# david8862/tf-keras-deeplabv3p-model-set

Measured on AMD Instinct MI355X. Metric: images/sec (513x513, 21-class) MobileNetV2-DeepLabV3+ OS=16 training step, higher is better.
Workload: dtype f32

## Files before the change

include/dl3p.h:

```cpp
#ifndef DL3P_H_
#define DL3P_H_

#include <stddef.h>
#include <stdint.h>

#ifdef __cplusplus
extern "C" {
#endif

#define DL3P_VERSION 100

enum {
  DL3P_OK = 0,
  DL3P_EINVAL = -1,
  DL3P_EUNSUPPORTED = -2,
  DL3P_ELAUNCH = -3,
  DL3P_EWORKSPACE = -4
};

enum { DL3P_ACT_NONE = 0, DL3P_ACT_RELU = 1, DL3P_ACT_RELU6 = 2, DL3P_ACT_HSWISH = 3, DL3P_ACT_HSIGMOID = 4 };

#define DL3P_MAX_STAT_ROWS 2048

int dl3p_version(void);
// ... 247 lines not shown
                                 int M, int K, int N, void* stream);
int dl3p_dwconv2d_bwd_weight_slabs(const float* x, int ldx, const float* in_scale, const float* in_shift, int in_act,
                                   const float* dy, int lddy, float* workspace, size_t workspace_bytes, int* rows_out,
                                   int N, int H, int W, int C, int k, int stride, int rate, int pad_t, int pad_l,
                                   int Ho, int Wo, void* stream);
int dl3p_stem_conv_bwd_weight_slabs(const float* x, int ldx, const float* dy, int lddy, float* workspace,
                                    size_t workspace_bytes, int* rows_out, int N, int H, int W, int Cout, int pad_t,
                                    int pad_l, int Ho, int Wo, void* stream);
int dl3p_stem_conv_bwd_weight_slabs_bn(const float* x, int ldx, const float* g, int ldg, const float* z, int ldz,
                                       const float* bn_scale, const float* bn_shift, int bn_act, const float* save_mean,
                                       const float* save_invstd, const float* coef, float* workspace, size_t workspace_bytes,
                                       int* rows_out, int N, int H, int W, int Cout, int pad_t, int pad_l, int Ho, int Wo,
                                       void* stream);
int dl3p_conv2d_gemm_bwd_weight_slabs(const float* x, int ldx, const float* in_scale, const float* in_shift, int in_act,
                                      const float* dy, int lddy, float* workspace, size_t workspace_bytes, int* rows_out,
                                      int N, int H, int W, int Cin, int Cout, int k, int stride, int rate,
                                      int pad_t, int pad_l, int Ho, int Wo, void* stream);
int dl3p_pwconv_bwd_weight_bn_supported(int M, int K, int N);
int dl3p_pwconv_bwd_weight_slabs_bn(const float* x, int ldx, const float* in_scale, const float* in_shift, int in_act,
                                    const float* g, int ldg, const float* z, int ldz, const float* bn_scale,
                                    const float* bn_shift, int bn_act, const float* save_mean, const float* save_invstd,
                                    const float* coef, float* dz, int lddz, float* workspace, size_t workspace_bytes,
                                    int* rows_out, int M, int K, int N, void* stream);
int dl3p_dw_upsampled_input(const float* up_x, int up_ld, int up_h, int up_w, int up_C, void* stream);
int dl3p_dw_upsampled_input_supported(int role, int N, int H, int W, int C, int up_C, int k, int stride, int rate, int pad_t, int pad_l,
                                      int Ho, int Wo);
int dl3p_dwconv2d_bwd_weight_bn_supported(int N, int H, int W, int C, int k, int stride, int rate, int pad_t, int pad_l,
                                          int Ho, int Wo);
int dl3p_dwconv2d_bwd_weight_slabs_bn(const float* x, int ldx, const float* in_scale, const float* in_shift, int in_act,
                                      const float* g, int ldg, const float* z, int ldz, const float* bn_scale,
                                      const float* bn_shift, int bn_act, const float* save_mean, const float* save_invstd,
                                      const float* coef, float* dz, int lddz, float* workspace, size_t workspace_bytes,
                                      int* rows_out, int N, int H, int W, int C, int k, int stride, int rate, int pad_t,
                                      int pad_l, int Ho, int Wo, void* stream);
int dl3p_pwconv_bwd_weight_slabs_bf16(const void* x, int ldx, const float* in_scale, const float* in_shift, int in_act,
                                      const void* dy, int lddy, int dy_is_f32, float* workspace, size_t workspace_bytes,
                                      int* rows_out, int M, int K, int N, void* stream);
int dl3p_dwconv2d_bwd_weight_slabs_bf16(const void* x, int ldx, const float* in_scale, const float* in_shift, int in_act,
                                        const void* dy, int lddy, float* workspace, size_t workspace_bytes, int* rows_out,
                                        int N, int H, int W, int C, int k, int stride, int rate, int pad_t, int pad_l,
                                        int Ho, int Wo, void* stream);

int dl3p_sgd_momentum(float* w, float* v, const float* g, size_t n, const float* lr_dev, float momentum,
                      float l2, float grad_scale, const float* l2_elem, const float* lr_scale_elem, void* stream);

int dl3p_adam_step(float* w, float* m, float* v, const float* g, size_t n, const float* lr_dev,
// ... 182 lines not shown
```

tf-keras-deeplabv3p-model-set_amd/_lib.py:

```python
import ctypes
import os
import re

HERE = os.path.dirname(os.path.abspath(__file__))
HEADER = os.path.join(HERE, '..', 'include', 'dl3p.h')
LIBPATH = os.path.join(HERE, 'libdl3p.so')

_CT = {
    'const float*': ctypes.c_void_p, 'float*': ctypes.c_void_p,
    'const double*': ctypes.c_void_p, 'double*': ctypes.c_void_p,
    'const int64_t*': ctypes.c_void_p, 'int64_t*': ctypes.c_void_p,
    'void*': ctypes.c_void_p, 'const void*': ctypes.c_void_p, 'void**': ctypes.POINTER(ctypes.c_void_p), 'int*': ctypes.POINTER(ctypes.c_int), 'unsigned long long*': ctypes.c_void_p, 'int32_t*': ctypes.c_void_p, 'uint32_t*': ctypes.c_void_p, 'const unsigned char*': ctypes.c_void_p, 'unsigned char*': ctypes.c_void_p, 'uint8_t*': ctypes.c_void_p, 'const uint8_t*': ctypes.c_void_p, 'const int*': ctypes.c_void_p, 'float*': ctypes.c_void_p,
    'int': ctypes.c_int, 'float': ctypes.c_float, 'double': ctypes.c_double,
    'size_t': ctypes.c_size_t, 'uint64_t': ctypes.c_uint64,
    'const char*': ctypes.c_char_p, 'void': None,
}


def parse_header(path=HEADER):
    src = open(path).read()
    src = re.sub(r'/\*.*?\*/', '', src, flags=re.S)
    src = re.sub(r'^\s*#.*$', '', src, flags=re.M)
    src = re.sub(r'\benum\s*\{[^}]*\}\s*;', '', src)
    src = src.replace('extern "C" {', '')
# ... 13 lines not shown
    return protos


class Dl3pError(RuntimeError):
    pass


class Lib:
    def __init__(self, path=LIBPATH):
        if not os.path.exists(path):
            raise ImportError(
                'libdl3p.so not found at %s -- build it with `python __graft_entry__.py` '
                '(there is no CPU fallback for the HIP path)' % path)
        import torch
        self.cdll = ctypes.CDLL(path)
        self.protos = parse_header()
        for name, (ret, args) in self.protos.items():
            fn = getattr(self.cdll, name)
            fn.restype = _CT[ret]
            fn.argtypes = [_CT[a] for a in args]
            setattr(self, name[len('dl3p_'):], self._wrap(name, fn, ret))

    def _wrap(self, name, fn, ret):
        if ret != 'int' or name in ('dl3p_version', 'dl3p_device_cus', 'dl3p_head_train_supported', 'dl3p_head_train_rows_supported', 'dl3p_stem_conv_supported', 'dl3p_conv2d_gemm_supported', 'dl3p_reduce_rows_variant', 'dl3p_reduce_rows_block_elements', 'dl3p_pwconv_bwd_weight_bn_supported', 'dl3p_dwconv2d_bwd_weight_bn_supported', 'dl3p_pwconv_sb_supported', 'dl3p_pwconv_sb_pays', 'dl3p_pwconv_bwd_data_sb_apply_supported', 'dl3p_conv2d_gemm_sb_supported', 'dl3p_conv2d_gemm_sb_pays', 'dl3p_irb_supported', 'dl3p_pwconv_fwd_splitk_plan', 'dl3p_irb_bwd_supported', 'dl3p_get_option', 'dl3p_irb_get_plan', 'dl3p_irb_cov_rows_max', 'dl3p_dw_upsampled_input_supported', 'dl3p_conv_narrow_supported', 'dl3p_ghost_fwd_supported', 'dl3p_deconv2x2_supported', 'dl3p_grad_clip_block_elements'):
            return fn
        err = self.cdll.dl3p_last_error_string
        err.restype = ctypes.c_char_p

        def call(*a):
            rc = fn(*a)
            if rc != 0:
                raise Dl3pError('%s failed (%d): %s' % (name, rc, err().decode()))
            return rc
        call.raw = fn
        call.__name__ = name
        return call


_lib = None


def lib():
    global _lib
    if _lib is None:
        _lib = Lib(os.environ['DL3P_LIB_OVERRIDE']) if os.environ.get('DL3P_LIB_OVERRIDE') else Lib()
    return _lib
```

tf-keras-deeplabv3p-model-set_amd/csrc/options.h:

```cpp
#pragma once
#include "common.h"

enum OptGet { GET_NONE, GET_SET, GET_LATCHED, GET_LATCHED_GE0, GET_RESOLVED };

#define DL3P_OPTION_TABLE(X)                                                                                                  \
                                                                    \
  X(PW_SMALL_MIN_ROWS, GET_NONE, "pw_small_min_rows", "DL3P_PW_SMALL_MIN_ROWS", 1 << 17, -1, v < 0 ? (1 << 17) : v)           \
                                \
  X(GEMM_NT, GET_NONE, "gemm_nt", nullptr, 0, 0, (v >= 1 && v <= 8) ? v : 0)                                                  \
              \
  X(GEMM_MI, GET_NONE, "gemm_mi", "DL3P_GEMM_MI", 0, 0, (v == 1 || v == 2) ? v : 0)                                           \
  X(GEMM_PER_CU, GET_NONE, "gemm_per_cu", "DL3P_GEMM_PER_CU", 0, 0, v > 0 ? v : 0)                                            \
                                                                \
  X(GEMM_TUNED, GET_NONE, "gemm_tuned", "DL3P_GEMM_TUNED", 1, -1, v ? 1 : 0)                                                  \
                   \
  X(SB_PIPE, GET_RESOLVED, "sb_pipe", "DL3P_SB_PIPE", 0, -1, v ? 1 : 0)                                                       \
                                                        \
  X(SPLIT_WGRAD, GET_LATCHED, "split_wgrad", "DL3P_SPLIT_WGRAD", env_int("DL3P_SPLIT_GEMM", 1), -1, v ? 1 : 0)                \
           \
  X(SPLIT_WGRAD_TILE, GET_NONE, "split_wgrad_tile", nullptr, -1, -1, (v >= 0 && v <= 4) ? v : -1)                             \
  X(SPLIT_WGRAD_PER_CU, GET_NONE, "split_wgrad_per_cu", nullptr, 0, 0, v > 0 ? v : 0)                                         \
                                                        \
  X(SPLITK, GET_SET, "splitk", "DL3P_SPLITK", -1, -1, v)                                                                      \
                     \
  X(SB_WM, GET_NONE, "sb_wm", nullptr, 0, 0, (v >= -1 && v <= 2) ? v : 0)                                                     \
  X(SB_NT, GET_NONE, "sb_nt", nullptr, 0, 0, (v == 8 || v == 12 || v == 16) ? v : 0)                                          \
                                       \
  X(SB_RS, GET_SET, "sb_rs", "DL3P_SB_RS", -1, -1, v < 0 ? -1 : (v ? 1 : 0))                                                  \
                                        \
  X(SB3, GET_LATCHED_GE0, "sb3", "DL3P_SB3", -1, -1, v < 0 ? -1 : (v ? 1 : 0))                                                \
                                     \
  X(BF16_KG, GET_NONE, "bf16_kg", "DL3P_BF16_KG", 0, -1, (v == 0 || v == 1 || v == 2 || v == 4) ? v : -1)                     \
                        \
  X(CONV_SB, GET_SET, "conv_sb", "DL3P_CONV_SB", 1, -1, (v >= 0 && v <= 2) ? v : -1)                                          \
                                      \
  X(DW_PER_CU, GET_NONE, "dw_per_cu", nullptr, 0, 0, v > 0 ? v : 0)                                                           \
  X(DW_WANT, GET_NONE, "dw_want", "DL3P_DW_WANT", DL3P_NUM_CUS * 3 / 2, 0, v > 0 ? v : 0)                                     \
  X(DW_MAXTH, GET_NONE, "dw_maxth", "DL3P_DW_MAXTH", 16, 0, v > 0 ? v : 0)                                                    \
  X(DW_TW, GET_NONE, "dw_tw", nullptr, 0, 0, (v == 2 || v == 4) ? v : 0)                                                      \
  X(DW_TUNED, GET_NONE, "dw_tuned", "DL3P_DW_TUNED", 1, -1, v ? 1 : 0)                                                        \
                                                                                                               \
  X(WGRAD_TILE, GET_NONE, "wgrad_tile", "DL3P_WGRAD_TILE", -1, -1, (v >= 0 && v <= 3) ? v : -1)                               \
  X(WGRAD_PER_CU, GET_NONE, "wgrad_per_cu", "DL3P_WGRAD_PER_CU", 4, 0, v > 0 ? v : 0)

enum Opt {
#define X(id, get, name, env, def, unset, norm) OPT_##id,
  DL3P_OPTION_TABLE(X)
#undef X
  OPT_COUNT
};

struct OptState { int set, env; bool env_read; };
extern OptState g_opt[OPT_COUNT];
int opt_env_read(Opt id);

static constexpr int k_opt_unset[OPT_COUNT] = {
#define X(id, get, name, env, def, unset, norm) unset,
// ... 8 lines not shown
```

tf-keras-deeplabv3p-model-set_amd/executor.py:

```python
import collections
import contextlib
import ctypes
import zlib
import numpy as np
import torch

from ._lib import lib
from .exec_options import GHOST_ON_BY_DEFAULT, ExecOptions
from .graph import ACT_NONE, ACT_RELU

MAX_ROWS = 2048
GHOST_DEFAULT = {(16, 8), (16, 24), (48, 12), (24, 36), (72, 12)}
GHOST_MIN_ROWS = 0

CONV_KINDS = ('conv_pw', 'conv_dense', 'conv_dw')
(R_IRB_EXPAND, R_IRB_DW, R_GHOST_PW, R_GHOST_DW, R_PW, R_DW, R_STEM, R_NARROW, R_GEMM, R_IM2COL) = (
    'irb_expand', 'irb_dw', 'ghost_pw', 'ghost_dw', 'pw', 'dw', 'stem', 'narrow', 'gemm', 'im2col')
NO_FRONT_SUMS = (None, 0, None, None, ACT_NONE, None, None, None, None)
Folded = collections.namedtuple('Folded', 'g ldg z ldz scale shift act mean invstd coef')
FoldedDg = collections.namedtuple('FoldedDg', Folded._fields + ('dz', 'lddz'))


def split_gemm_enabled():
    return ExecOptions.from_env().split_gemm
# ... 1231 lines not shown
    def _begin_backward(self, T):
        T.ws, T.wsb = self.workspace.data_ptr(), self.workspace.numel() * 4
        for op in self.g.ops:
            if getattr(op, 'b', None) is not None and self._bias_grad(op) is None:
                self.store.view(op.b, self.store.G).zero_()
        bucket_edges = self._bucket_edges() if self.dist is not None else {}
        T.defer = self.sync_bn
        T.fuse = self._bn_fusion_map()
        if self.bf16:
            T.fuse = {c: b for c, b in T.fuse.items() if c.kind == 'conv_pw' and self._rows(c) > 64 and self.opts.bf16_fuse_bn_bwd}
        T.stage_off = self._sync_total
        T.readers = self._bn_readers()
        T.bn_of = {id(o.z): o for o in self.g.ops if o.kind == 'bn'}
        T.fuse_add = self._bn_fusion_through_adds(T.readers) if not self.bf16 else {}
        T.batch = self.opts.batched_wgrad
        T.batch_wgrad = T.batch and not T.defer
        if T.batch_wgrad and not self.bf16:
            need = max([self._rows(op) * (op.cout if op.kind == 'conv_pw' else op.c) for op in self.g.ops
                        if op.kind in ('conv_pw', 'conv_dw') and op not in self._irb_expand] or [0])
            T.dz_scratch = torch.zeros(need + 64, **self.f32)
        if T.batch:
            slab_need = 0
            for op in self.g.ops:
                if op.kind in CONV_KINDS and op.layer.trainable and self._slab_bytes(op):
                    slab_need += (self._slab_bytes(op) + 255) // 256 * 256
            T.slab_ws = torch.zeros(slab_need // 4 + 64, **self.f32) if slab_need else None
        return bucket_edges

    def _wgrad(self, P, fn, *args):
        if self._bt.defer:
            self._bt.deferred.append((fn, args, P.ctx))
        else:
            P.k(fn, *args)

    def _slab_region(self, nbytes):
        T = self._bt
        region = T.slab_ws.data_ptr() + 4 * T.slab_off
        T.slab_off += ((nbytes + 255) // 256 * 256) // 4
        return region

    def _wgrad_slabs(self, P, fn, n, dst, nbytes, before, after, up=None):
        T, L = self._bt, self.L
        region = self._slab_region(nbytes)

        def issue(P2):
            rows = ctypes.c_int(0)
            if up is not None:
                P2.k(L.dw_upsampled_input, *up)
# ... 13 lines not shown
            for op2 in later:
                if (op2.kind == 'bn' and op2 not in T.bn_done and op2.z.requires_grad and op2.bn.layer.trainable
                        and T.readers.get(op2) and T.readers[op2] <= T.processed and op2 not in T.fuse.values()):
                    self._bn_backward_done(P, op2)

    def _bn_backward_done(self, P, bn_op, fused_rows=None):
        with P.at(_op_label(bn_op)):
            self._bn_backward(P, bn_op, fused_rows=fused_rows)
        self._bt.bn_done.add(bn_op)

    def _front_sums_done(self, P, front, front_add, rows):
        if front is not None:
            self._bn_backward_done(P, front, fused_rows=rows)
        elif front_add is not None:
            self._bt.presums[front_add] = rows

    def _conv_backward(self, P, op):
        T, out, xt = self._bt, op.out, op.x.tensor
        dz, lddz = self.tptr(out, True), out.ld
        need_gx = xt.requires_grad or xt.root.requires_grad
        sums_left = None
        if op.kind == 'conv_pw' and out.id in T.folded_dg:
            dz, lddz, sums_left = self._dgrad_folded(P, op)
        if op.layer.trainable and T.batch and self._slab_bytes(op):
            dz, lddz = self._wgrad_slab(P, op, dz, lddz, need_gx)
        elif op.layer.trainable:
            self._wgrad_plain(P, op, dz, lddz)
        if sums_left is not None:
            self._front_sums_done(P, *sums_left)
        elif need_gx:
            self._dgrad(P, op, dz, lddz)

    def _dgrad_folded(self, P, op):
        f = self._bt.folded_dg.pop(op.out.id)
        gp, ldg, acc = self._gbuf_acc(op.x)
        wsp, pitch = self.store.sb_ptr(op, False)
        front, front_add = self._front_bn(op)
        rows = ctypes.c_int(0)
        sums = self._front_sums(front or front_add, self.partials if front is not None else self.partials2, rows)
        P.k(self.L.pwconv_bwd_data_sb_apply, *f, wsp, pitch, gp, ldg, acc, *self._mkn(op), *sums)
        return f.dz, f.lddz, (front, front_add, rows.value)

    def _wgrad_slab(self, P, op, dz, lddz, need_gx):
        T, L = self._bt, self.L
        r = self._bwd_route(op)
        x = self.vargs(op.x)
        f = T.folded.pop(op.out.id, None)
        if f is not None and r != R_STEM:
            dz, lddz = (T.dz_scratch.data_ptr(), op.cout if r == R_PW else op.c) if need_gx else (None, 0)
        bn = f is not None
        before = (*x, *f, dz, lddz) if bn else (*x, dz, lddz)
        if r == R_PW:
            fn, n, after = (L.pwconv_bwd_weight_slabs_bn if bn else L.pwconv_bwd_weight_slabs), op.cin * op.cout, self._mkn(op)
        elif r == R_DW:
# ... 393 lines not shown
            if fused_rows is None:
                P.k(L.bn_bwd_reduce_bf16 if self.bf16 else L.bn_bwd_reduce, g, ldg, zp, ldz, sp, hp, bn.act, mean, invstd,
                    part, ctypes.byref(rows), M, bn.C)
            P.k(L.bn_bwd_finalize, part, rows.value, None, bn.C, float(M), st.ptr(lp['gamma']),
                invstd, sp, 0, st.ptr(lp['gamma'], G), st.ptr(lp['beta'], G), coef)
            if self.sync_bn:
                off = T.stage_off
                T.stage_off += 2 * bn.C
                P.k(L.bn_reduce_partials, part, rows.value, 2 * bn.C, self.sync_stage[off:].data_ptr())
                T.pending.append((op, off, P.ctx))
                T.sync_g[op] = (g, ldg)
                return
        if not frozen and op in self._irb_bn:
            return
        if not frozen and self._folds_apply_dgrad(op):
            T.folded_dg[z.id] = FoldedDg(g, ldg, zp, ldz, sp, hp, bn.act, mean, invstd, coef, dzo, lddzo)
            return
        if not frozen and self._folds_apply(op):
            T.folded[z.id] = Folded(g, ldg, zp, ldz, sp, hp, bn.act, mean, invstd, coef)
            T.dz_not_kept.add(z.root.id)
            return
        P.k(L.bn_bwd_apply_bf16 if self.bf16 else L.bn_bwd_apply, g, ldg, zp, ldz, sp, hp, bn.act, mean, invstd, coef, dzo,
            lddzo, 0, M, bn.C)

    def _folds_apply_dgrad(self, bn_op):
        conv = getattr(bn_op, 'producer', None)
        if (self.bf16 or self.sync_bn or self.dist is not None or conv is None or conv.kind != 'conv_pw' or conv.out is not bn_op.z
                or self.opts.fold_apply == 'off' or not self.opts.fold_apply_dgrad
                or conv in self._irb_expand):
            return False
        xt = conv.x.tensor
        if not (xt.requires_grad or xt.root.requires_grad):
            return False
        M = self._rows(conv)
        front, front_add = self._front_bn(conv)
        front = front or front_add
        vt = getattr(conv.x, 'view_grad', None)
        ldg = vt.ld if vt is not None else xt.ld
        if M * max(xt.ld, ldg, bn_op.z.ld, conv.cout, front.z.ld if front is not None else 0) * 4 >= 2 ** 32:
            return False
        if not self.L.pwconv_bwd_data_sb_apply_supported(M, conv.cin, conv.cout, bn_op.bn.act, 1 if front is not None else 0):
            return False
        return self._use_sb(conv, False, front is not None)

    def _folds_apply(self, bn_op):
        conv = getattr(bn_op, 'producer', None)
# ... 355 lines not shown
```

tf-keras-deeplabv3p-model-set_amd/ops.py:

```python
import ctypes
import torch

from ._lib import lib, Dl3pError

ACT_NONE, ACT_RELU, ACT_RELU6, ACT_HSWISH, ACT_HSIGMOID = 0, 1, 2, 3, 4
MAX_STAT_ROWS = 2048


def _stream():
    return torch.cuda.current_stream().cuda_stream


def _pl(t):
    if t is None:
        return None, 0
    if not t.is_cuda or t.dtype != torch.float32:
        raise Dl3pError('dl3p ops need float32 tensors on the HIP device (got %s on %s)' % (t.dtype, t.device))
    if t.stride(-1) != 1:
        raise Dl3pError('channel dim must be contiguous')
    ld = t.stride(-2) if t.dim() >= 2 else t.shape[-1]
    for d in range(t.dim() - 2):
        if t.shape[d + 1] > 0 and t.stride(d) != t.stride(d + 1) * t.shape[d + 1]:
            raise Dl3pError('rows are not evenly strided: %s %s' % (tuple(t.shape), t.stride()))
    return t.data_ptr(), ld
# ... 192 lines not shown
    dp, ldd = _pl(dy)
    lib().pwconv_bwd_weight(xp, ldx, _p(in_scale), _p(in_shift), in_act, dp, ldd, _p(gw), _p(gb), _p(ws),
                            ws.numel() * 4, M, K, Nn, _stream())
    return (gw, gb) if with_bias else gw


def pwconv_bwd_weight_bn(x, g, z, bn, act, in_scale=None, in_shift=None, in_act=ACT_NONE, want_dz=True):
    K, Nn = x.shape[-1], g.shape[-1]
    M = _rows(x)
    need = lib().pwconv_bwd_weight_workspace(M, K, Nn)
    ws = torch.empty(need // 4, dtype=torch.float32, device=x.device)
    gw = torch.empty((K, Nn), dtype=torch.float32, device=x.device)
    dz = torch.empty(g.shape, dtype=torch.float32, device=x.device) if want_dz else None
    xp, ldx = _pl(x)
    gp, ldg = _pl(g)
    zp, ldz = _pl(z)
    dp, ldd = _pl(dz)
    rows = ctypes.c_int(0)
    lib().pwconv_bwd_weight_slabs_bn(xp, ldx, _p(in_scale), _p(in_shift), in_act, gp, ldg, zp, ldz, _p(bn.scale), _p(bn.shift),
                                     act, _p(bn.mean), _p(bn.invstd), _p(bn.coef), dp, ldd or 0, _p(ws), ws.numel() * 4,
                                     ctypes.byref(rows), M, K, Nn, _stream())
    lib().reduce_rows(_p(ws), rows.value, K * Nn, _p(gw), 0, _stream())
    return gw, dz


def conv2d_fwd(x, w, stride=1, rate=1, padding='same', in_scale=None, in_shift=None, in_act=ACT_NONE, out=None,
               partials=None):
    N, H, W, Cin = x.shape
    k, _, _, Cout = w.shape
    Ho, Wo, pt, pl = conv_geometry(H, W, k, stride, rate, padding)
    y = out if out is not None else torch.empty((N, Ho, Wo, Cout), dtype=torch.float32, device=x.device)
    xp, ldx = _pl(x)
    yp, ldy = _pl(y)
    rows = ctypes.c_int(0)
    lib().conv2d_fwd(xp, ldx, _p(in_scale), _p(in_shift), in_act, _p(w), yp, ldy, _p(partials), ctypes.byref(rows),
                     N, H, W, Cin, Cout, k, stride, rate, pt, pl, Ho, Wo, _stream())
    return (y, rows.value) if partials is not None else y


def conv2d_bwd_weight(x, dy, k, stride=1, rate=1, padding='same', in_scale=None, in_shift=None, in_act=ACT_NONE):
    N, H, W, Cin = x.shape
    Cout = dy.shape[-1]
    Ho, Wo, pt, pl = conv_geometry(H, W, k, stride, rate, padding)
    need = lib().conv2d_bwd_weight_workspace(N, Ho, Wo, Cin, Cout, k)
    ws = torch.empty(need // 4, dtype=torch.float32, device=x.device)
    gw = torch.empty((k, k, Cin, Cout), dtype=torch.float32, device=x.device)
# ... 1050 lines not shown
```

Baseline: 1360.

## Fuse narrow pointwise conv backward: weight grad, data grad and BN stats in one kernel

Adds a fused HIP kernel for pointwise convolutions with small output channel counts. In one pass over the rows it applies the own BN backward, accumulates the weight gradient (and optional bias gradient) into per-block slabs, computes the input gradient with the weights held in LDS, and gathers the front BN statistics. The executor routes eligible conv_pw ops to it by default. This drops separate wgrad and dgrad launches and repeated reads of activations and gradients, at the cost of more LDS and register pressure and extra slab workspace.

```diff
diff --git a/include/dl3p.h b/include/dl3p.h
--- a/include/dl3p.h
+++ b/include/dl3p.h
@@ -293,6 +293,17 @@
                                     const float* bn_shift, int bn_act, const float* save_mean, const float* save_invstd,
                                     const float* coef, float* dz, int lddz, float* workspace, size_t workspace_bytes,
                                     int* rows_out, int M, int K, int N, void* stream);
+int dl3p_pwconv_bwd_narrow_supported(int M, int K, int N, int in_act, int own_act, int has_front, int has_bias, int accumulate,
+                                     int ld_max);
+int dl3p_pwconv_bwd_narrow_pays(int M, int K, int N);
+size_t dl3p_pwconv_bwd_narrow_workspace(int M, int K, int N, int ldw);
+int dl3p_pwconv_bwd_narrow(const float* z_in, int ldx, const float* in_scale, const float* in_shift, int in_act,
+                           const float* g, int ldg, const float* z_own, int ldz_own, const float* bn_scale,
+                           const float* bn_shift, int bn_act, const float* save_mean, const float* save_invstd,
+                           const float* coef, const float* w, int ldw, float* gx, int ldgx, int accumulate,
+                           const float* front_mean, const float* front_invstd, float* front_partials,
+                           int* front_rows_out, int with_bias, float* workspace, size_t workspace_bytes,
+                           int* rows_out, int M, int K, int N, void* stream);
 int dl3p_dw_upsampled_input(const float* up_x, int up_ld, int up_h, int up_w, int up_C, void* stream);
 int dl3p_dw_upsampled_input_supported(int role, int N, int H, int W, int C, int up_C, int k, int stride, int rate, int pad_t, int pad_l,
                                       int Ho, int Wo);
diff --git a/tf-keras-deeplabv3p-model-set_amd/_lib.py b/tf-keras-deeplabv3p-model-set_amd/_lib.py
--- a/tf-keras-deeplabv3p-model-set_amd/_lib.py
+++ b/tf-keras-deeplabv3p-model-set_amd/_lib.py
@@ -59,7 +59,7 @@
             setattr(self, name[len('dl3p_'):], self._wrap(name, fn, ret))
 
     def _wrap(self, name, fn, ret):
-        if ret != 'int' or name in ('dl3p_version', 'dl3p_device_cus', 'dl3p_head_train_supported', 'dl3p_head_train_rows_supported', 'dl3p_stem_conv_supported', 'dl3p_conv2d_gemm_supported', 'dl3p_reduce_rows_variant', 'dl3p_reduce_rows_block_elements', 'dl3p_pwconv_bwd_weight_bn_supported', 'dl3p_dwconv2d_bwd_weight_bn_supported', 'dl3p_pwconv_sb_supported', 'dl3p_pwconv_sb_pays', 'dl3p_pwconv_bwd_data_sb_apply_supported', 'dl3p_conv2d_gemm_sb_supported', 'dl3p_conv2d_gemm_sb_pays', 'dl3p_irb_supported', 'dl3p_pwconv_fwd_splitk_plan', 'dl3p_irb_bwd_supported', 'dl3p_get_option', 'dl3p_irb_get_plan', 'dl3p_irb_cov_rows_max', 'dl3p_dw_upsampled_input_supported', 'dl3p_conv_narrow_supported', 'dl3p_ghost_fwd_supported', 'dl3p_deconv2x2_supported', 'dl3p_grad_clip_block_elements'):
+        if ret != 'int' or name in ('dl3p_version', 'dl3p_device_cus', 'dl3p_head_train_supported', 'dl3p_head_train_rows_supported', 'dl3p_stem_conv_supported', 'dl3p_conv2d_gemm_supported', 'dl3p_reduce_rows_variant', 'dl3p_reduce_rows_block_elements', 'dl3p_pwconv_bwd_weight_bn_supported', 'dl3p_pwconv_bwd_narrow_supported', 'dl3p_pwconv_bwd_narrow_pays', 'dl3p_dwconv2d_bwd_weight_bn_supported', 'dl3p_pwconv_sb_supported', 'dl3p_pwconv_sb_pays', 'dl3p_pwconv_bwd_data_sb_apply_supported', 'dl3p_conv2d_gemm_sb_supported', 'dl3p_conv2d_gemm_sb_pays', 'dl3p_irb_supported', 'dl3p_pwconv_fwd_splitk_plan', 'dl3p_irb_bwd_supported', 'dl3p_get_option', 'dl3p_irb_get_plan', 'dl3p_irb_cov_rows_max', 'dl3p_dw_upsampled_input_supported', 'dl3p_conv_narrow_supported', 'dl3p_ghost_fwd_supported', 'dl3p_deconv2x2_supported', 'dl3p_grad_clip_block_elements'):
             return fn
         err = self.cdll.dl3p_last_error_string
         err.restype = ctypes.c_char_p
diff --git a/tf-keras-deeplabv3p-model-set_amd/csrc/options.h b/tf-keras-deeplabv3p-model-set_amd/csrc/options.h
--- a/tf-keras-deeplabv3p-model-set_amd/csrc/options.h
+++ b/tf-keras-deeplabv3p-model-set_amd/csrc/options.h
@@ -33,6 +33,8 @@
   X(BF16_KG, GET_NONE, "bf16_kg", "DL3P_BF16_KG", 0, -1, (v == 0 || v == 1 || v == 2 || v == 4) ? v : -1)                     \
                         \
   X(CONV_SB, GET_SET, "conv_sb", "DL3P_CONV_SB", 1, -1, (v >= 0 && v <= 2) ? v : -1)                                          \
+                                                                                                              \
+  X(PW_NARROW, GET_SET, "pw_narrow", "DL3P_PW_NARROW", 1, -1, (v >= 0 && v <= 2) ? v : -1)                                    \
                                       \
   X(DW_PER_CU, GET_NONE, "dw_per_cu", nullptr, 0, 0, v > 0 ? v : 0)                                                           \
   X(DW_WANT, GET_NONE, "dw_want", "DL3P_DW_WANT", DL3P_NUM_CUS * 3 / 2, 0, v > 0 ? v : 0)                                     \
diff --git a/tf-keras-deeplabv3p-model-set_amd/csrc/pw_narrow_bwd.hip b/tf-keras-deeplabv3p-model-set_amd/csrc/pw_narrow_bwd.hip
--- /dev/null
+++ b/tf-keras-deeplabv3p-model-set_amd/csrc/pw_narrow_bwd.hip
@@ -0,0 +1,439 @@
+#include <algorithm>
+#include <initializer_list>
+#include "common.h"
+#include "options.h"
+
+typedef float f32x4 __attribute__((ext_vector_type(4)));
+
+struct NarrowParams {
+  const float* X; int ldx; const float* scale; const float* shift; int act;
+  const float* G; int ldg;
+  const float* Z; int ldz;
+  const float* b_scale; const float* b_shift; const float* b_mean; const float* b_invstd; const float* b_coef; int b_act;
+  const float* W; int ldw;
+  float* GX; int ldgx;
+  const float* f_mean; const float* f_invstd; float* partials;
+  float* slabs; float* bias_slabs;
+  int M, K, N, S, R;
+};
+
+template <int KT, int NTN, int WAVES, bool BNA, bool BNB, bool BIAS>
+__global__ __launch_bounds__(64 * WAVES, (KT == 4 && (NTN == 2 || (BNA && BNB))) ? 2 : 3) void pw_narrow_bwd_kernel(NarrowParams p) {
+  constexpr int KS = 16 * KT, NP = 16 * NTN;
+  constexpr int XP = KS + 4, DP = NP + 4;
+  constexpr int WAVE_FLOATS = 16 * (XP + DP);
+  extern __shared__ __attribute__((aligned(16))) float nb_lds[];
+  const int WP = p.K + 4;
+  float* Wt = nb_lds;
+  float* sc_s = Wt + NP * WP;
+  float* sh_s = sc_s + p.K;
+  float* mu_s = sh_s + p.K;
+  float* is_s = mu_s + (BNB ? p.K : 0);
+  float* cf_s = is_s + (BNB ? p.K : 0);
+  float* wave0 = cf_s + (BNA ? 5 * NP : 0);
+  const int nthreads = blockDim.x;
+  const int t = threadIdx.x, l = t & 63, w = t >> 6, l15 = l & 15, q = l >> 4;
+  const int stream = w / p.S, slice = w - stream * p.S;
+  const int k0 = slice * KS;
+  float* Xs = wave0 + w * WAVE_FLOATS;
+  float* Ds = Xs + 16 * XP;
+  for (int idx = t; idx < NP * p.K; idx += nthreads) {
+    const int k = idx / NP, n = idx - k * NP;
+    Wt[n * WP + k] = n < p.N ? p.W[(size_t)k * p.ldw + n] : 0.f;
+  }
+  for (int i = t; i < p.K; i += nthreads) {
+    sc_s[i] = p.scale ? p.scale[i] : 1.f;
+    sh_s[i] = p.scale ? p.shift[i] : 0.f;
+    if (BNB) { mu_s[i] = p.f_mean[i]; is_s[i] = p.f_invstd[i]; }
+  }
+  if (BNA) {
+    for (int i = t; i < NP; i += nthreads) {
+      const bool in = i < p.N;
+      const float c0 = in ? p.b_coef[i] : 0.f, c1 = in ? p.b_coef[p.N + i] : 0.f, c2 = in ? p.b_coef[2 * p.N + i] : 0.f;
+      const float bc = in ? c0 * p.b_invstd[i] * c2 : 0.f;
+      cf_s[i] = c0;
+      cf_s[NP + i] = bc;
+      cf_s[2 * NP + i] = in ? bc * p.b_mean[i] - c0 * c1 : 0.f;
+      cf_s[3 * NP + i] = (in && p.b_scale) ? p.b_scale[i] : 1.f;
+      cf_s[4 * NP + i] = (in && p.b_shift) ? p.b_shift[i] : 0.f;
+    }
+  }
+  __syncthreads();
+
+  uint32_t xg[KT], gg[NTN], zg[BNA ? NTN : 1];
+  bool nok[NTN][4];
+#pragma unroll
+  for (int kt = 0; kt < KT; ++kt) xg[kt] = (uint32_t)(k0 + 16 * kt + 4 * q) * 4u;
+#pragma unroll
+  for (int nt = 0; nt < NTN; ++nt) {
+    const int n = 16 * nt + 4 * q;
+    gg[nt] = (uint32_t)(n < p.N ? n : 0) * 4u;
+    if (BNA) zg[nt] = gg[nt];
+#pragma unroll
+    for (int e = 0; e < 4; ++e) nok[nt][e] = n + e < p.N;
+  }
+  const float act_lo = p.act == DL3P_ACT_NONE ? -DL3P_INF : 0.f;
+  const float act_hi = (p.act == DL3P_ACT_NONE || p.act == DL3P_ACT_RELU) ? DL3P_INF : 6.f;
+
+  f32x4 acc[KT][NTN];
+#pragma unroll
+  for (int a = 0; a < KT; ++a)
+#pragma unroll
+    for (int b = 0; b < NTN; ++b) acc[a][b] = (f32x4){0.f, 0.f, 0.f, 0.f};
+  float4 st_s[BNB ? KT : 1], st_q[BNB ? KT : 1], bsum[BIAS ? NTN : 1];
+  if (BNB) {
+#pragma unroll
+    for (int i = 0; i < KT; ++i) { st_s[i] = zero4(); st_q[i] = zero4(); }
+  }
+  if (BIAS) {
+#pragma unroll
+    for (int i = 0; i < NTN; ++i) bsum[i] = zero4();
+  }
+
+  const int ntiles = (p.M + 15) >> 4;
+  const int nstreams = gridDim.x * p.R;
+  const int gs = blockIdx.x * p.R + stream;
+  const char* Xb = reinterpret_cast<const char*>(p.X);
+  const char* Gb = reinterpret_cast<const char*>(p.G);
+  const char* Zb = reinterpret_cast<const char*>(p.Z);
+  char* Ob = reinterpret_cast<char*>(p.GX);
+  float4 rx[KT], rg[NTN], rz[BNA ? NTN : 1];
+#define NB_PREFETCH_X(tile_)                                                                                   \
+  {                                                                                                            \
+    const uint32_t xb0 = (uint32_t)min(((tile_) << 4) + l15, p.M - 1) * (uint32_t)p.ldx * 4u;                  \
+    _Pragma("unroll") for (int i = 0; i < KT; ++i) rx[i] = *reinterpret_cast<const float4*>(Xb + (xb0 + xg[i]));   \
+  }
+#define NB_PREFETCH_G(tile_)                                                                                   \
+  {                                                                                                            \
+    const uint32_t prow = (uint32_t)min(((tile_) << 4) + l15, p.M - 1);                                        \
+    const uint32_t gb0 = prow * (uint32_t)p.ldg * 4u;                                                          \
+    _Pragma("unroll") for (int i = 0; i < NTN; ++i) rg[i] = *reinterpret_cast<const float4*>(Gb + (gb0 + gg[i]));  \
+    if (BNA) {                                                                                                 \
+      const uint32_t zb0 = prow * (uint32_t)p.ldz * 4u;                                                        \
+      _Pragma("unroll") for (int i = 0; i < NTN; ++i) rz[i] = *reinterpret_cast<const float4*>(Zb + (zb0 + zg[i])); \
+    }                                                                                                          \
+  }
+  NB_PREFETCH_X(min(gs, ntiles - 1))
+  NB_PREFETCH_G(min(gs, ntiles - 1))
+  for (int tile = gs; tile < ntiles; tile += nstreams) {
+    const int m0 = tile << 4;
+    const bool row_ok = m0 + l15 < p.M;
+    int cq = 4 * q;
+    asm volatile("" : "+v"(cq));
+    float4 xh[BNB ? KT : 1];
+    uint32_t dmask = 0;
+#pragma unroll
+    for (int kt = 0; kt < KT; ++kt) {
+      const float4 s4 = *reinterpret_cast<const float4*>(&sc_s[k0 + 16 * kt + cq]);
+      const float4 h4 = *reinterpret_cast<const float4*>(&sh_s[k0 + 16 * kt + cq]);
+      const float4 u = fma4(rx[kt], s4, h4);
+      const float4 v = make_float4(__builtin_amdgcn_fmed3f(u.x, act_lo, act_hi), __builtin_amdgcn_fmed3f(u.y, act_lo, act_hi),
+                                   __builtin_amdgcn_fmed3f(u.z, act_lo, act_hi), __builtin_amdgcn_fmed3f(u.w, act_lo, act_hi));
+      *reinterpret_cast<float4*>(&Xs[l15 * XP + 16 * kt + 4 * q]) = row_ok ? v : zero4();
+      if (BNB) {
+        const float4 mu = *reinterpret_cast<const float4*>(&mu_s[k0 + 16 * kt + cq]);
+        const float4 is = *reinterpret_cast<const float4*>(&is_s[k0 + 16 * kt + cq]);
+        const float4 zv = rx[kt];
+        xh[kt] = make_float4((zv.x - mu.x) * is.x, (zv.y - mu.y) * is.y, (zv.z - mu.z) * is.z, (zv.w - mu.w) * is.w);
+        dmask |= ((u.x > act_lo && u.x < act_hi) ? 1u : 0u) << (4 * kt);
+        dmask |= ((u.y > act_lo && u.y < act_hi) ? 1u : 0u) << (4 * kt + 1);
+        dmask |= ((u.z > act_lo && u.z < act_hi) ? 1u : 0u) << (4 * kt + 2);
+        dmask |= ((u.w > act_lo && u.w < act_hi) ? 1u : 0u) << (4 * kt + 3);
+        asm volatile("" : "+v"(xh[kt].x), "+v"(xh[kt].y), "+v"(xh[kt].z), "+v"(xh[kt].w));
+      }
+    }
+    if (BNB) asm volatile("" : "+v"(dmask));
+    float dz[NTN][4];
+#pragma unroll
+    for (int nt = 0; nt < NTN; ++nt) {
+      float4 v = rg[nt];
+      if (BNA) {
+        const int cf = 16 * nt + cq;
+        const float4 a4 = *reinterpret_cast<const float4*>(&cf_s[cf]);
+        const float4 c4 = *reinterpret_cast<const float4*>(&cf_s[NP + cf]);
+        const float4 d4 = *reinterpret_cast<const float4*>(&cf_s[2 * NP + cf]);
+        const float4 s4 = *reinterpret_cast<const float4*>(&cf_s[3 * NP + cf]);
+        const float4 h4 = *reinterpret_cast<const float4*>(&cf_s[4 * NP + cf]);
+        const float4 z = rz[nt];
+        const float4 u = fma4(z, s4, h4);
+        const int act = p.b_act;
+        v = make_float4(fmaf(a4.x, v.x * act_grad(u.x, act), fmaf(-c4.x, z.x, d4.x)),
+                        fmaf(a4.y, v.y * act_grad(u.y, act), fmaf(-c4.y, z.y, d4.y)),
+                        fmaf(a4.z, v.z * act_grad(u.z, act), fmaf(-c4.z, z.z, d4.z)),
+                        fmaf(a4.w, v.w * act_grad(u.w, act), fmaf(-c4.w, z.w, d4.w)));
+      }
+      dz[nt][0] = (row_ok && nok[nt][0]) ? v.x : 0.f;
+      dz[nt][1] = (row_ok && nok[nt][1]) ? v.y : 0.f;
+      dz[nt][2] = (row_ok && nok[nt][2]) ? v.z : 0.f;
+      dz[nt][3] = (row_ok && nok[nt][3]) ? v.w : 0.f;
+      const float4 d4v = make_float4(dz[nt][0], dz[nt][1], dz[nt][2], dz[nt][3]);
+      *reinterpret_cast<float4*>(&Ds[l15 * DP + 16 * nt + 4 * q]) = d4v;
+      if (BIAS) bsum[nt] = add4(bsum[nt], d4v);
+    }
+    NB_PREFETCH_X(min(tile + nstreams, ntiles - 1))
+    __builtin_amdgcn_sched_barrier(0);
+    {
+      float b[NTN][4];
+#pragma unroll
+      for (int nt = 0; nt < NTN; ++nt)
+#pragma unroll
+        for (int j = 0; j < 4; ++j) b[nt][j] = Ds[(4 * q + j) * DP + nt * 16 + l15];
+#pragma unroll
+      for (int kt = 0; kt < KT; ++kt) {
+        float a[4];
+#pragma unroll
+        for (int j = 0; j < 4; ++j) a[j] = Xs[(4 * q + j) * XP + kt * 16 + l15];
+#pragma unroll
+        for (int nt = 0; nt < NTN; ++nt)
+#pragma unroll
+          for (int j = 0; j < 4; ++j)
+            acc[kt][nt] = __builtin_amdgcn_mfma_f32_16x16x4f32(b[nt][j], a[j], acc[kt][nt], 0, 0, 0);
+      }
+    }
+    f32x4 gacc[KT];
+#pragma unroll
+    for (int kt = 0; kt < KT; ++kt) {
+      gacc[kt] = (f32x4){0.f, 0.f, 0.f, 0.f};
+#pragma unroll
+      for (int nt = 0; nt < NTN; ++nt)
+#pragma unroll
+        for (int j = 0; j < 4; ++j)
+          gacc[kt] = __builtin_amdgcn_mfma_f32_16x16x4f32(Wt[(nt * 16 + 4 * q + j) * WP + k0 + kt * 16 + l15], dz[nt][j], gacc[kt], 0, 0, 0);
+    }
+    __builtin_amdgcn_sched_barrier(0);
+    NB_PREFETCH_G(min(tile + nstreams, ntiles - 1))
+#pragma unroll
+    for (int kt = 0; kt < KT; ++kt) {
+      const float4 o = make_float4(gacc[kt][0], gacc[kt][1], gacc[kt][2], gacc[kt][3]);
+      if (BNB) {
+        const float4 d = make_float4((dmask >> (4 * kt)) & 1u ? o.x : 0.f, (dmask >> (4 * kt + 1)) & 1u ? o.y : 0.f,
+                                     (dmask >> (4 * kt + 2)) & 1u ? o.z : 0.f, (dmask >> (4 * kt + 3)) & 1u ? o.w : 0.f);
+        st_s[kt] = add4(st_s[kt], d);
+        st_q[kt] = fma4(d, xh[kt], st_q[kt]);
+      }
+      *reinterpret_cast<float4*>(&Xs[l15 * XP + 16 * kt + 4 * q]) = o;
+    }
+    const uint32_t ob0 = ((uint32_t)m0 * (uint32_t)p.ldgx + (uint32_t)k0) * 4u;
+    const int rows_here = p.M - m0;
+#pragma unroll
+    for (int i = 0; i < KT; ++i) {
+      const int f = l + 64 * i;
+      const int r = f / (KS / 4), c = f - r * (KS / 4);
+      if (r < rows_here)
+        st4(reinterpret_cast<float*>(Ob + (ob0 + ((uint32_t)r * (uint32_t)p.ldgx + (uint32_t)c * 4u) * 4u)),
+            *reinterpret_cast<const float4*>(&Xs[r * XP + c * 4]));
+    }
+  }
+#undef NB_PREFETCH_X
+#undef NB_PREFETCH_G
+
+  __syncthreads();
+  int t_end = threadIdx.x;
+  asm volatile("" : "+v"(t_end));
+  const int te = t_end, le = te & 63, we = te >> 6, l15e = le & 15, qe = le >> 4;
+  const int streame = we / p.S, slicee = we - streame * p.S;
+  const int k0e = slicee * KS;
+  float4* red = reinterpret_cast<float4*>(nb_lds);
+  if (streame > 0) {
+#pragma unroll
+    for (int kt = 0; kt < KT; ++kt)
+#pragma unroll
+      for (int nt = 0; nt < NTN; ++nt)
+        red[(((streame - 1) * p.S + slicee) * KT * NTN + kt * NTN + nt) * 64 + le] =
+            make_float4(acc[kt][nt][0], acc[kt][nt][1], acc[kt][nt][2], acc[kt][nt][3]);
+  }
+  __syncthreads();
+  if (streame == 0) {
+    float* slab = p.slabs + (size_t)blockIdx.x * p.K * p.ldw;
+#pragma unroll
+    for (int kt = 0; kt < KT; ++kt)
+#pragma unroll
+      for (int nt = 0; nt < NTN; ++nt) {
+        float4 v = make_float4(acc[kt][nt][0], acc[kt][nt][1], acc[kt][nt][2], acc[kt][nt][3]);
+        for (int r = 1; r < p.R; ++r) v = add4(v, red[(((r - 1) * p.S + slicee) * KT * NTN + kt * NTN + nt) * 64 + le]);
+        const int k = k0e + kt * 16 + l15e, n = nt * 16 + qe * 4;
+        if (n < p.ldw) st4(slab + (size_t)k * p.ldw + n, v);
+      }
+  }
+  if (BNB) {
+    float4* S4 = reinterpret_cast<float4*>(nb_lds);
+    const int k4 = p.K >> 2;
+#pragma unroll
+    for (int which = 0; which < 2; ++which) {
+      __syncthreads();
+#pragma unroll
+      for (int kt = 0; kt < KT; ++kt) S4[(streame * 16 + l15e) * k4 + ((k0e + 16 * kt) >> 2) + qe] = which ? st_q[kt] : st_s[kt];
+      __syncthreads();
+      if (te < k4) {
+        float4 sum = zero4();
+        for (int ww = 0; ww < p.R; ++ww)
+          for (int r = 0; r < 16; ++r) sum = add4(sum, S4[(ww * 16 + r) * k4 + te]);
+        st4(p.partials + ((size_t)blockIdx.x * 2 + which) * p.K + 4 * te, sum);
+      }
+    }
+  }
+  if (BIAS) {
+    __syncthreads();
+    float* bred = nb_lds;
+#pragma unroll
+    for (int nt = 0; nt < NTN; ++nt) {
+      float bv[4] = {bsum[nt].x, bsum[nt].y, bsum[nt].z, bsum[nt].w};
+#pragma unroll
+      for (int e = 0; e < 4; ++e) {
+        float s1 = bv[e];
+#pragma unroll
+        for (int d = 1; d < 16; d <<= 1) s1 += __shfl_xor(s1, d);
+        if (l15e == 0 && slicee == 0) bred[streame * NP + 16 * nt + 4 * qe + e] = s1;
+      }
+    }
+    __syncthreads();
+    for (int i = te; i < p.ldw; i += nthreads) {
+      float sum = bred[i];
+      for (int r = 1; r < p.R; ++r) sum += bred[r * NP + i];
+      p.bias_slabs[(size_t)blockIdx.x * p.ldw + i] = sum;
+    }
+  }
+}
+
+struct NarrowPlan { int kt, ntn, S, R, grid; size_t lds; };
+
+static int narrow_kt(int K) {
+  if (K == 32) return 2;
+  if (K % 48 == 0 && K <= 192) return 3;
+  if (K % 64 == 0 && K <= 256) return 4;
+  return 0;
+}
+
+static bool narrow_plan(int M, int K, int N, bool bna, bool bnb, NarrowPlan* pl) {
+  const int kt = narrow_kt(K);
+  if (M <= 0 || N < 1 || N > 32 || !kt) return false;
+  pl->kt = kt;
+  pl->ntn = N <= 16 ? 1 : 2;
+  pl->S = K / (16 * kt);
+  pl->R = pl->S <= 3 ? 4 : 1;
+  static const int per_cu_env = env_int("DL3P_PW_NARROW_PER_CU", 0);
+  const int per_cu = per_cu_env > 0 ? per_cu_env : (pl->R == 1 && kt == 3 ? 3 : 2);
+  int g = ceil_div(M, 16) / (pl->R * 2);
+  g = std::min(g, DL3P_NUM_CUS * per_cu);
+  g = std::min(g, DL3P_MAX_STAT_ROWS);
+  pl->grid = std::max(g, 1);
+  const int np = 16 * pl->ntn, ks = 16 * kt, waves = pl->S * pl->R;
+  const size_t stage = (size_t)np * (K + 4) + 2 * K + (bnb ? 2 * K : 0) + (bna ? 5 * np : 0) + (size_t)waves * 16 * (ks + 4 + np + 4);
+  const size_t red = std::max({(size_t)4 * (pl->R - 1) * pl->S * kt * pl->ntn * 64, (size_t)pl->R * 16 * K, (size_t)pl->R * np});
+  pl->lds = sizeof(float) * std::max(stage, red);
+  return true;
+}
+
+template <int KT, int NTN, int WAVES, bool BNA, bool BNB, bool BIAS>
+static void launch_narrow(const NarrowParams& p, const NarrowPlan& pl, hipStream_t st) {
+  static size_t attr_lds = 0;
+  if (pl.lds > attr_lds) {
+    (void)hipFuncSetAttribute(reinterpret_cast<const void*>(pw_narrow_bwd_kernel<KT, NTN, WAVES, BNA, BNB, BIAS>),
+                              hipFuncAttributeMaxDynamicSharedMemorySize, (int)pl.lds);
+    attr_lds = pl.lds;
+  }
+  dl3p_launch(pw_narrow_bwd_kernel<KT, NTN, WAVES, BNA, BNB, BIAS>, dim3(pl.grid), dim3(64 * WAVES), pl.lds, st, p);
+}
+
+template <int KT, int NTN, int WAVES>
+static void launch_narrow_modes(const NarrowParams& p, const NarrowPlan& pl, bool bna, bool bnb, bool bias, hipStream_t st) {
+  if (bias) {
+    if (bnb) launch_narrow<KT, NTN, WAVES, false, true, true>(p, pl, st);
+    else launch_narrow<KT, NTN, WAVES, false, false, true>(p, pl, st);
+  } else if (bna) {
+    if (bnb) launch_narrow<KT, NTN, WAVES, true, true, false>(p, pl, st);
+    else launch_narrow<KT, NTN, WAVES, true, false, false>(p, pl, st);
+  } else {
+    if (bnb) launch_narrow<KT, NTN, WAVES, false, true, false>(p, pl, st);
+    else launch_narrow<KT, NTN, WAVES, false, false, false>(p, pl, st);
+  }
+}
+
+template <int NTN>
+static bool launch_narrow_shape(const NarrowParams& p, const NarrowPlan& pl, bool bna, bool bnb, bool bias, hipStream_t st) {
+  switch (pl.kt * 100 + pl.S * pl.R) {
+    case 204: launch_narrow_modes<2, NTN, 4>(p, pl, bna, bnb, bias, st); return true;
+    case 304: launch_narrow_modes<3, NTN, 4>(p, pl, bna, bnb, bias, st); return true;
+    case 308: launch_narrow_modes<3, NTN, 8>(p, pl, bna, bnb, bias, st); return true;
+    case 312: launch_narrow_modes<3, NTN, 12>(p, pl, bna, bnb, bias, st); return true;
+    case 404: launch_narrow_modes<4, NTN, 4>(p, pl, bna, bnb, bias, st); return true;
+    case 408: launch_narrow_modes<4, NTN, 8>(p, pl, bna, bnb, bias, st); return true;
+    default: return false;
+  }
+}
+
+static bool narrow_act_ok(int act) { return act == DL3P_ACT_NONE || act == DL3P_ACT_RELU || act == DL3P_ACT_RELU6; }
+
+extern "C" int dl3p_pwconv_bwd_narrow_supported(int M, int K, int N, int in_act, int own_act, int has_front, int has_bias,
+                                                int accumulate, int ld_max) {
+  NarrowPlan pl;
+  if (!narrow_plan(M, K, N, own_act >= 0, has_front != 0, &pl)) return 0;
+  if (accumulate || !narrow_act_ok(in_act) || own_act > DL3P_ACT_HSIGMOID) return 0;
+  if (own_act >= 0 && has_bias) return 0;
+  if (ld_max < 0 || (unsigned long long)M * (unsigned long long)std::max(ld_max, std::max(K, 32)) * 4ull >= (1ull << 32)) return 0;
+  return 1;
+}
+
+extern "C" int dl3p_pwconv_bwd_narrow_pays(int M, int K, int N) {
+  const int mode = opt(OPT_PW_NARROW);
+  if (mode == 0) return 0;
+  if (mode == 2) return 1;
+  NarrowPlan pl;
+  return M >= (1 << 17) && narrow_plan(M, K, N, false, false, &pl) && pl.R == 4;
+}
+
+extern "C" size_t dl3p_pwconv_bwd_narrow_workspace(int M, int K, int N, int ldw) {
+  NarrowPlan pl;
+  if (!narrow_plan(M, K, N, false, false, &pl) || ldw < N || ldw > 16 * pl.ntn) return 0;
+  return (size_t)pl.grid * ((size_t)K * ldw + ldw) * sizeof(float);
+}
+
+extern "C" int dl3p_pwconv_bwd_narrow(const float* z_in, int ldx, const float* in_scale, const float* in_shift, int in_act,
+                                      const float* g, int ldg, const float* z_own, int ldz_own, const float* bn_scale,
+                                      const float* bn_shift, int bn_act, const float* save_mean, const float* save_invstd,
+                                      const float* coef, const float* w, int ldw, float* gx, int ldgx, int accumulate,
+                                      const float* front_mean, const float* front_invstd, float* front_partials,
+                                      int* front_rows_out, int with_bias, float* workspace, size_t workspace_bytes,
+                                      int* rows_out, int M, int K, int N, void* stream) {
+  const char* fn = "dl3p_pwconv_bwd_narrow";
+  const bool bna = z_own != nullptr, bnb = front_partials != nullptr;
+  const int n4 = (N + 3) / 4 * 4;
+  DL3P_CHECK_ARG(z_in && g && w && gx && workspace && rows_out && aligned16(z_in) && aligned16(g) && aligned16(w) && aligned16(gx) &&
+                 aligned16(workspace), "%s: null or misaligned operand", fn);
+  DL3P_CHECK_ARG(M > 0 && K > 0 && N > 0 && ldx >= K && ldgx >= K && ldg >= n4 && ldw >= N && ldw <= (N <= 16 ? 16 : 32) && ldx % 4 == 0 && ldgx % 4 == 0 &&
+                 ldg % 4 == 0 && ldw % 4 == 0, "%s: bad layout (M=%d K=%d N=%d ldx=%d ldgx=%d ldg=%d ldw=%d)", fn, M, K, N, ldx, ldgx, ldg, ldw);
+  DL3P_CHECK_ARG((in_scale == nullptr) == (in_shift == nullptr), "%s: in_scale and in_shift come together", fn);
+  if (bna)
+    DL3P_CHECK_ARG(aligned16(z_own) && ldz_own >= n4 && ldz_own % 4 == 0 && save_mean && save_invstd && coef && N % 4 == 0,
+                   "%s: bad BatchNorm-apply operands", fn);
+  if (bnb)
+    DL3P_CHECK_ARG(in_scale && front_mean && front_invstd && front_rows_out, "%s: bad front BatchNorm operands", fn);
+  const int ld_max = std::max({ldx, ldgx, ldg, bna ? ldz_own : 0});
+  DL3P_CHECK_ARG(dl3p_pwconv_bwd_narrow_supported(M, K, N, in_act, bna ? bn_act : -1, bnb, with_bias, accumulate, ld_max),
+                 "%s: not served (M=%d K=%d N=%d in_act=%d own_act=%d bias=%d accumulate=%d, or operands of 4 GiB or more)", fn, M, K,
+                 N, in_act, bna ? bn_act : -1, with_bias, accumulate);
+  NarrowPlan pl;
+  narrow_plan(M, K, N, bna, bnb, &pl);
+  const size_t need = dl3p_pwconv_bwd_narrow_workspace(M, K, N, ldw);
+  if (workspace_bytes < need) {
+    dl3p_set_error("%s: workspace %zu < %zu bytes", fn, workspace_bytes, need);
+    return DL3P_EWORKSPACE;
+  }
+  NarrowParams p = {};
+  p.X = z_in; p.ldx = ldx; p.scale = in_scale; p.shift = in_shift; p.act = in_act;
+  p.G = g; p.ldg = ldg;
+  p.Z = z_own; p.ldz = ldz_own; p.b_scale = bn_scale; p.b_shift = bn_shift; p.b_mean = save_mean; p.b_invstd = save_invstd;
+  p.b_coef = coef; p.b_act = bn_act;
+  p.W = w; p.ldw = ldw; p.GX = gx; p.ldgx = ldgx;
+  p.f_mean = front_mean; p.f_invstd = front_invstd; p.partials = front_partials;
+  p.slabs = workspace; p.bias_slabs = workspace + (size_t)pl.grid * K * ldw;
+  p.M = M; p.K = K; p.N = N; p.S = pl.S; p.R = pl.R;
+  hipStream_t st = (hipStream_t)stream;
+  const bool bias = with_bias != 0;
+  const bool launched = pl.ntn == 1 ? launch_narrow_shape<1>(p, pl, bna, bnb, bias, st) : launch_narrow_shape<2>(p, pl, bna, bnb, bias, st);
+  DL3P_CHECK_ARG(launched, "%s: no instantiation for K=%d", fn, K);
+  DL3P_CHECK_LAUNCH(fn);
+  *rows_out = pl.grid;
+  if (bnb) *front_rows_out = pl.grid;
+  return DL3P_OK;
+}
diff --git a/tf-keras-deeplabv3p-model-set_amd/executor.py b/tf-keras-deeplabv3p-model-set_amd/executor.py
--- a/tf-keras-deeplabv3p-model-set_amd/executor.py
+++ b/tf-keras-deeplabv3p-model-set_amd/executor.py
@@ -1277,8 +1277,8 @@
         if T.batch:
             slab_need = 0
             for op in self.g.ops:
-                if op.kind in CONV_KINDS and op.layer.trainable and self._slab_bytes(op):
-                    slab_need += (self._slab_bytes(op) + 255) // 256 * 256
+                if op.kind in CONV_KINDS and op.layer.trainable:
+                    slab_need += (max(self._slab_bytes(op), self._narrow_bwd_bytes(op)) + 255) // 256 * 256
             T.slab_ws = torch.zeros(slab_need // 4 + 64, **self.f32) if slab_need else None
         return bucket_edges
 
@@ -1338,6 +1338,9 @@
         sums_left = None
         if op.kind == 'conv_pw' and out.id in T.folded_dg:
             dz, lddz, sums_left = self._dgrad_folded(P, op)
+        elif self._narrow_bwd(op):
+            self._backward_narrow(P, op, dz, lddz)
+            return
         if op.layer.trainable and T.batch and self._slab_bytes(op):
             dz, lddz = self._wgrad_slab(P, op, dz, lddz, need_gx)
         elif op.layer.trainable:
@@ -1346,6 +1349,28 @@
             self._front_sums_done(P, *sums_left)
         elif need_gx:
             self._dgrad(P, op, dz, lddz)
+
+    def _backward_narrow(self, P, op, dz, lddz):
+        T, L, st = self._bt, self.L, self.store
+        f = T.folded.pop(op.out.id, None)
+        own = tuple(f) if f is not None else (dz, lddz, None, 0, None, None, ACT_NONE, None, None, None)
+        gp, ldg, acc = self._gbuf_acc(op.x)
+        front, _ = self._front_bn(op)
+        rows, frows = ctypes.c_int(0), ctypes.c_int(0)
+        sums = (None, None, None, None)
+        if front is not None:
+            aux = self.bn_aux[front.bn]
+            sums = (aux['mean'].data_ptr(), aux['invstd'].data_ptr(), self.partials.data_ptr(), ctypes.byref(frows))
+        b = self._bias_grad(op)
+        M, K, N = self._mkn(op)
+        nbytes = self._narrow_bwd_bytes(op)
+        region = self._slab_region(nbytes)
+        P.k(L.pwconv_bwd_narrow, *self.vargs(op.x), *own, st.ptr(op.w), N, gp, ldg, acc, *sums, 1 if b is not None else 0, region,
+            nbytes, ctypes.byref(rows), M, K, N)
+        T.jobs.append((region, st.ptr(op.w, st.G), rows.value, K * N))
+        if b is not None:
+            T.jobs.append((region + 4 * rows.value * K * N, st.ptr(b, st.G), rows.value, N))
+        self._front_sums_done(P, front, None, frows.value)
 
     def _dgrad_folded(self, P, op):
         f = self._bt.folded_dg.pop(op.out.id)
@@ -1785,6 +1810,48 @@
             return
         P.k(L.bn_bwd_apply_bf16 if self.bf16 else L.bn_bwd_apply, g, ldg, zp, ldz, sp, hp, bn.act, mean, invstd, coef, dzo,
             lddzo, 0, M, bn.C)
+
+    def _narrow_bwd_static(self, op):
+        T = self._bt
+        if (op.kind != 'conv_pw' or self.bf16 or self.sync_bn or self.dist is not None or not op.layer.trainable or not T.batch_wgrad
+                or self._bwd_route(op) != R_PW or self._rows(op) <= 64):
+            return None
+        v, xt = op.x, op.x.tensor
+        if not (xt.requires_grad or xt.root.requires_grad) or getattr(v, 'view_grad', None) is not None:
+            return None
+        front, front_add = self._front_bn(op)
+        if front_add is not None:
+            return None
+        if front is not None and (front.z is not xt or v.group is None or v.act != front.bn.act
+                                  or self.vargs(v)[2:4] != self._bn_coeffs(front.bn)):
+            return None
+        M, K, N = self._mkn(op)
+        has_bias = self._bias_grad(op) is not None
+        ld_max = max(xt.ld, op.out.ld, N)
+        if not self.L.pwconv_bwd_narrow_supported(M, K, N, v.act, -1, 1 if front is not None else 0, 1 if has_bias else 0, 0, ld_max):
+            return None
+        if not self.L.pwconv_bwd_narrow_pays(M, K, N):
+            return None
+        return front, has_bias
+
+    def _narrow_bwd_bytes(self, op):
+        return self.L.pwconv_bwd_narrow_workspace(*self._mkn(op), op.cout) if self._narrow_bwd_static(op) is not None else 0
+
+    def _narrow_bwd(self, op):
+        st = self._narrow_bwd_static(op)
+        if st is None:
+            return False
+        T, xt = self._bt, op.x.tensor
+        if xt.id in T.written or (xt.base is not None and xt.base.id in T.written):
+            return False
+        f = T.folded.get(op.out.id)
+        if f is not None:
+            M, K, N = self._mkn(op)
+            front, has_bias = st
+            ld_max = max(xt.ld, op.out.ld, N, f.ldg, f.ldz)
+            return bool(self.L.pwconv_bwd_narrow_supported(M, K, N, op.x.act, f.act, 1 if front is not None else 0,
+                                                           1 if has_bias else 0, 0, ld_max))
+        return True
 
     def _folds_apply_dgrad(self, bn_op):
         conv = getattr(bn_op, 'producer', None)
diff --git a/tf-keras-deeplabv3p-model-set_amd/ops.py b/tf-keras-deeplabv3p-model-set_amd/ops.py
--- a/tf-keras-deeplabv3p-model-set_amd/ops.py
+++ b/tf-keras-deeplabv3p-model-set_amd/ops.py
@@ -238,6 +238,33 @@
                                      ctypes.byref(rows), M, K, Nn, _stream())
     lib().reduce_rows(_p(ws), rows.value, K * Nn, _p(gw), 0, _stream())
     return gw, dz
+
+
+def pwconv_bwd_narrow(x, g, w, n=None, in_scale=None, in_shift=None, in_act=ACT_NONE, z_own=None, bn=None, own_act=ACT_NONE,
+                      front_mean=None, front_invstd=None, partials=None, with_bias=False, out=None, accumulate=False):
+    K, ldw = w.shape[-2], w.shape[-1]
+    Nn = ldw if n is None else n
+    M = _rows(x)
+    need = lib().pwconv_bwd_narrow_workspace(M, K, Nn, ldw)
+    ws = torch.empty(max(need, 16) // 4, dtype=torch.float32, device=x.device)
+    gx = out if out is not None else torch.empty(tuple(x.shape[:-1]) + (K,), dtype=torch.float32, device=x.device)
+    xp, ldx = _pl(x)
+    gp, ldg = _pl(g)
+    zp, ldz = _pl(z_own)
+    op, ldo = _pl(gx)
+    b = bn if z_own is not None else None
+    rows, frows = ctypes.c_int(0), ctypes.c_int(0)
+    lib().pwconv_bwd_narrow(xp, ldx, _p(in_scale), _p(in_shift), in_act, gp, ldg, zp, ldz, _p(b and b.scale), _p(b and b.shift),
+                            own_act, _p(b and b.mean), _p(b and b.invstd), _p(b and b.coef), _p(w), ldw, op, ldo, int(accumulate),
+                            _p(front_mean), _p(front_invstd), _p(partials), ctypes.byref(frows), int(with_bias), _p(ws),
+                            ws.numel() * 4, ctypes.byref(rows), M, K, Nn, _stream())
+    gw = torch.empty((K, ldw), dtype=torch.float32, device=x.device)
+    lib().reduce_rows(_p(ws), rows.value, K * ldw, _p(gw), 0, _stream())
+    gb = None
+    if with_bias:
+        gb = torch.empty((ldw,), dtype=torch.float32, device=x.device)
+        lib().reduce_rows(_p(ws) + 4 * rows.value * K * ldw, rows.value, ldw, _p(gb), 0, _stream())
+    return gw, gb, gx, frows.value
 
 
 def conv2d_fwd(x, w, stride=1, rate=1, padding='same', in_scale=None, in_shift=None, in_act=ACT_NONE, out=None,
```

New measurement: 1369, median of 6. No clear change (+0.6%).
